# whabacivch/GC-SLAM

Measured on AMD Instinct MI355X. Metric: scans/sec (14-step pipeline) at 64k pts/scan, higher is better.
Workload: dtype f64

## Files before the change

gc-slam_amd/csrc/gcs_atlas.cpp:

```cpp
#include "gcs_atlas.h"

#include <math.h>

#include <algorithm>
#include <cmath>
#include <thread>
#include <vector>

#include "gcs_math.h"

namespace gcs {
namespace atlas {

void fibonacci(int B, double* dirs) {
  const double pi = 3.141592653589793;
  const double golden = pi * (1.0 + sqrt(5.0));
  for (int i = 0; i < B; ++i) {
    double idx = (double)i + 0.5;
    double phi = acos(1.0 - (2.0 * idx) / (double)B);
    double theta = golden * idx;
    double x = sin(phi) * cos(theta), y = sin(phi) * sin(theta), z = cos(phi);
    double n = sqrt(dot3_exact(x, y, z, x, y, z));
    double d = n + kEpsMass;
    dirs[3 * i] = x / d;
// ... 175 lines not shown
      L[k] = th[k].second;
      const double bd = cos(std::max(th[k].first - rc, 0.0)) + 1e-6;
      F[k] = std::nextafter((float)bd, 2.0f);
    }
  });
  width = 1;
  for (auto& L : lists) width = std::max(width, (int)L.size() + 1);
  width = (width + 3) & ~3;
  pools.assign((size_t)ncell * width, -1);
  for (int c = 0; c < ncell; ++c)
    std::copy(lists[c].begin(), lists[c].end(), pools.begin() + (size_t)c * width);
  if (bounds) {
    bounds->assign((size_t)ncell * width, -2.0f);
    for (int c = 0; c < ncell; ++c)
      std::copy(blists[c].begin(), blists[c].end(), bounds->begin() + (size_t)c * width);
  }
}

namespace {
uint64_t hilbert_d(uint32_t n, uint32_t x, uint32_t y) {
  uint64_t d = 0;
  for (uint32_t s = n / 2; s > 0; s /= 2) {
    uint32_t rx = (x & s) > 0, ry = (y & s) > 0;
    d += (uint64_t)s * s * ((3 * rx) ^ ry);
    if (ry == 0) {
      if (rx == 1) { x = s - 1 - x; y = s - 1 - y; }
      std::swap(x, y);
    }
  }
  return d;
// ... 51 lines not shown
```

gc-slam_amd/csrc/gcs_atlas.h:

```cpp
#pragma once
#include <stdint.h>

#include <vector>

namespace gcs {
namespace atlas {

void fibonacci(int B, double* dirs );
void knn(const double* dirs, int B, int K, int* out );
void nearest(const double* dirs, int B, int nq, const double* q, int* out);
void reverse(const int* knn, int B, int K, std::vector<int>& off, std::vector<int>& idx);
int grid_for_bins(int B);
void cell_pools(const double* dirs, int B, int G, std::vector<int>& pools, int& width,
                std::vector<float>* bounds = nullptr);

void hilbert_order(const double* dirs, int B, std::vector<int>& order);

int tile_sources(const std::vector<int>& rknn_off, const std::vector<int>& rknn, int B, int tile,
                 std::vector<int>& src_off, std::vector<int>& src, std::vector<uint16_t>& local);

}
}
```

gc-slam_amd/csrc/gcs_capi.cpp:

```cpp
#include "gcslam_hip.h"

#include <hip/hip_runtime.h>
#include <math.h>
#include <rccl/rccl.h>
#include <string.h>

#include <algorithm>
#include <atomic>
#include <sys/syscall.h>
#include <unistd.h>
#include <chrono>
#include <condition_variable>
#include <mutex>
#include <thread>
#include <string>
#include <vector>

#include "gcs_atlas.h"
#include "gcs_host.h"
#include "gcs_imu_odom_core.h"
#include "gcs_kernels.h"
#include "gcs_layout.h"
#include "gcs_live.h"
#include "gcs_math.h"
// ... 26 lines not shown
  clk::time_point T0, Tp, T1, Ts, T2;
};

struct gcs_ctx {
  gcs_config cfg{};
  int B = 0, cap = 0, K = 0, G = 0, pool_width = 0, ncell = 0, max_raw = 0;
  hipStream_t stream = nullptr;
  bool own_stream = false;
  std::string err;
  double* d_bin_dirs = nullptr;
  int* d_knn = nullptr;
  int* d_rknn_off = nullptr;
  int* d_rknn = nullptr;
  int* d_pools = nullptr;
  float* d_pool_bound = nullptr;
  std::vector<double> dirs_host;
  std::vector<int> knn_host;
  std::vector<int> order, inv;
  int* d_bin_ref = nullptr;
  int* d_tile_src_off = nullptr;
  int* d_tile_src = nullptr;
  uint16_t* d_rknn_local = nullptr;
  int max_tile_src = 0;
  int tile_bins = 64;
  int tile_shift = 6;
  PointRec* d_recs = nullptr;
  double* d_iz = nullptr;
  bool iz_valid = false;
  double *d_live_p0 = nullptr, *d_live_w = nullptr, *d_live_t = nullptr;
  gcs_scan_state* scan_st = nullptr;
// ... 300 lines not shown
    std::vector<uint16_t> local;
    c->max_tile_src = atlas::tile_sources(off, idx, B, c->tile_bins, src_off, src, local);
    if (c->max_tile_src > bins_max_tile_sources(c->tile_bins))
      return fail(c, GCS_ERR_ARG, "bin atlas too irregular for the tiled bin kernel (tile source list too long)");
    for (int b0 = 0; b0 < B; b0 += c->tile_bins)
      if (off[std::min(B, b0 + c->tile_bins)] - off[b0] > bins_max_tile_entries(c->tile_bins))
        return fail(c, GCS_ERR_ARG, "bin atlas too irregular for the tiled bin kernel (tile reverse-kNN list too long)");
    c->G = atlas::grid_for_bins(B);
    c->ncell = 6 * c->G * c->G;
    std::vector<float> pbound;
    atlas::cell_pools(c->dirs_host.data(), B, c->G, pools, c->pool_width, &pbound);
    if (int rc = upload(c, c->d_pool_bound, pbound)) return rc;
    for (int& id : pools)
      if (id >= 0) id = c->inv[id];
    if (int rc = upload(c, c->d_pools, pools)) return rc;
    HIPCHK(c, hipMemcpy(c->d_knn, knn_dev.data(), knn_dev.size() * sizeof(int), hipMemcpyHostToDevice));
    HIPCHK(c, hipMemcpy(c->d_rknn_off, off.data(), off.size() * sizeof(int), hipMemcpyHostToDevice));
    HIPCHK(c, hipMemcpy(c->d_rknn, idx.data(), idx.size() * sizeof(int), hipMemcpyHostToDevice));
    if (int rc = upload(c, c->d_tile_src_off, src_off)) return rc;
    if (int rc = upload(c, c->d_tile_src, src)) return rc;
    if (int rc = upload(c, c->d_rknn_local, local)) return rc;
  }
  HIPCHK(c, hipStreamSynchronize(nullptr));
  return GCS_OK;
}

int submit_budget(gcs_ctx* c, const BudgetArgs& ba, int nblk, hipStream_t s);

int stage_budget(gcs_ctx* c, const double* w, int n_raw, bool toggle = true, bool self = false) {
  if (n_raw < 0 || n_raw > c->max_raw) return fail(c, GCS_ERR_ARG, "n_points exceeds max_raw_points");
// ... 64 lines not shown
  a.cap = c->cap;
  a.t0 = t0;
  a.t1 = t1;
  memcpy(a.xi, xi, 6 * sizeof(double));
  memcpy(a.origin, c->cfg.lidar_origin, 3 * sizeof(double));
  a.tau = c->cfg.tau;
  a.bin_dirs = c->d_bin_dirs;
  a.n_bins = c->B;
  a.knn = c->d_knn;
  a.k = c->K;
  a.pools = c->d_pools;
  a.pool_bound = c->d_pool_bound;
  a.bin_ref = c->d_bin_ref;
  a.pool_width = c->pool_width;
  a.grid = c->G;
  a.recs = c->d_recs;
  a.keys = c->d_keys;
  a.slots = c->d_slots;
  a.counts = c->d_counts;
  if (c->use_direct) {
    a.members = c->d_members;
    a.capb = c->capb_eff;
    a.flags = c->d_flags;
    a.tile_shift = c->tile_shift;
    a.overflow = c->d_err + 2;
  }
  a.budget_partials = c->budget_self ? nullptr : c->d_partials;
  a.budget_blocks = c->budget_self ? 0 : c->budget_blocks;
  a.mass_rows = c->budget_self ? c->d_mass_rows : nullptr;
  c->recs_deferred = c->budget_self && c->cfg.mode == GCS_MODE_SCALE && !deskew_only;
// ... 17 lines not shown
  if (deskew_only) {
    a.n_bins = 0;
    a.nearest_out = nullptr;
    a.members = nullptr;
  }
  c->pts_blocks = points_blocks(c->cap, scale);
  c->pts_fold_pending = scale && fold_later;
  MirrorArgs mir{};
  if (to_host && !c->pts_fold_pending) {
    mir.mirror = c->d_scalars_mirror;
    mir.err = c->d_err;
    mir.seq = ++c->mirror_seq;
    mir.torn = c->mirror_torn;
  }
  HIPCHK(c, launch_points(a, scale, c->d_part_pts, c->pts_blocks, !c->pts_fold_pending, s, ev.e0, ev.e1,
                          c->legacy_points, mir));
  return GCS_OK;
}

BinKernelArgs bin_args(gcs_ctx* c) {
  BinKernelArgs b{};
  b.recs = c->d_recs;
  b.perm = c->d_perm;
  if (c->use_direct) {
    b.members = c->d_members;
    b.capb = c->capb_eff;
  }
  b.starts = c->d_starts;
  b.counts = c->d_counts;
  b.flags = c->d_flags;
  b.tile_dirty = c->d_tile_dirty;
// ... 446 lines not shown
  auto bad = [&](hipError_t e) {
    if (e != hipSuccess) {
      gcs_ctx_destroy(c);
      return true;
    }
    return false;
  };
  if (bad(hipSetDevice(cfg->device))) return GCS_ERR_HIP;
  if (bad(hipStreamCreateWithFlags(&c->stream, hipStreamNonBlocking))) return GCS_ERR_HIP;
  c->own_stream = true;
  if (bad(hipStreamCreateWithFlags(&c->push_stream, hipStreamNonBlocking))) return GCS_ERR_HIP;
  if (bad(hipEventCreateWithFlags(&c->ev_push, hipEventDisableTiming))) return GCS_ERR_HIP;
  if (bad(hipEventCreateWithFlags(&c->ev_stages, hipEventDisableTiming))) return GCS_ERR_HIP;
  if (const char* pt = getenv("GCSLAM_PUSH_THREAD")) c->push_async = atoi(pt) != 0;
  if (const char* sb = getenv("GCSLAM_SORTED_BUCKETS")) c->direct_buckets = atoi(sb) == 0;
  const size_t B = c->B, cap = c->cap;
  if (bad(hipMalloc(&c->d_bin_dirs, B * 4 * sizeof(double)))) return GCS_ERR_HIP;
  if (bad(hipMalloc(&c->d_recs, cap * sizeof(PointRec)))) return GCS_ERR_HIP;
  if (bad(hipMalloc(&c->d_iz, cap * sizeof(double)))) return GCS_ERR_HIP;
  if (bad(hipMalloc(&c->d_live_p0, 3 * cap * sizeof(double)))) return GCS_ERR_HIP;
  if (bad(hipMalloc(&c->d_live_w, cap * sizeof(double)))) return GCS_ERR_HIP;
  if (bad(hipMalloc(&c->d_live_t, cap * sizeof(double)))) return GCS_ERR_HIP;
  if (bad(hipMalloc(&c->d_nearest, cap * sizeof(int)))) return GCS_ERR_HIP;
  if (bad(hipMalloc(&c->d_scan, B * SF_COUNT * sizeof(double)))) return GCS_ERR_HIP;
  if (bad(hipMalloc(&c->d_map, B * MF_COUNT * sizeof(double)))) return GCS_ERR_HIP;
  if (bad(hipMalloc(&c->d_derived, B * MD_COUNT * sizeof(double)))) return GCS_ERR_HIP;
  if (bad(hipMemset(c->d_map, 0, B * MF_COUNT * sizeof(double)))) return GCS_ERR_HIP;
  if (bad(hipMemset(c->d_scan, 0, B * SF_COUNT * sizeof(double)))) return GCS_ERR_HIP;
  if (bad(hipMalloc(&c->d_touched, B))) return GCS_ERR_HIP;
  c->partials_len = std::max<size_t>({partials_need(kRedBlocks, 24), partials_need(pt_blocks(c->B), 13), partials_need(bins_scale_blocks(c->B, c->tile_bins), bins_partial_nv()),
// ... 90 lines not shown
}

int gcs_ctx_destroy(gcs_ctx* c) {
  if (!c) return GCS_OK;
  if (c->push_thread.joinable()) {
    (void)push_wait(c);
    {
      std::lock_guard<std::mutex> lk(c->push_mu);
      c->push_stop.store(true);
    }
    c->push_cv.notify_one();
    c->push_thread.join();
  }
  if (c->push_stream) (void)hipStreamSynchronize(c->push_stream);
  if (c->stream) (void)hipStreamSynchronize(c->stream);
  void* ptrs[] = {c->d_gate_xi, c->d_members, c->d_bin_dirs, c->d_knn, c->d_rknn_off, c->d_rknn, c->d_pools, c->d_pool_bound, c->d_recs, c->d_iz, c->d_live_p0, c->d_live_w, c->d_live_t, c->d_keys, c->d_slots,
                  c->d_sorted, c->d_nearest, c->d_counts, c->d_starts, c->d_perm, c->d_flags_buf[0], c->d_touched,
                  c->d_tile_dirty, c->d_tile_order, c->d_tile_work, c->d_bins_part, c->d_tickets,
                  c->d_bin_ref, c->d_tile_src_off, c->d_tile_src, c->d_rknn_local, c->d_part_pts, c->d_mass_rows, c->d_part_push, c->d_parse_flag,
                  c->d_scan, c->d_map, c->d_derived, c->d_bin_partials, c->d_partials, c->d_scalars};
  for (void* p : ptrs)
    if (p) (void)hipFree(p);
  if (c->h_scalars) (void)hipHostFree(c->h_scalars);
  if (c->d_err) (void)hipFree(c->d_err);
  if (c->h_gate) (void)hipHostFree(c->h_gate);
  if (c->h_preint_in) (void)hipHostFree(c->h_preint_in);
  if (c->h_preint_out) (void)hipHostFree(c->h_preint_out);
  if (c->comm_stream) {
    (void)hipStreamSynchronize(c->comm_stream);
    (void)hipStreamDestroy(c->comm_stream);
  }
// ... 153 lines not shown
  if (int rc = push_wait(c)) return rc;
  if (c->push_stream) HIPCHK(c, hipStreamSynchronize(c->push_stream));
  HIPCHK(c, hipStreamSynchronize(c->stream));
  const size_t B = c->B;
  int rc = 0;
  if ((rc = dev_fnv(c, c->d_scan, B * SF_COUNT * sizeof(double), &out[0]))) return rc;
  if ((rc = dev_fnv(c, c->d_map, B * MF_COUNT * sizeof(double), &out[1]))) return rc;
  if ((rc = dev_fnv(c, c->d_derived, B * MD_COUNT * sizeof(double), &out[2]))) return rc;
  if ((rc = dev_fnv(c, c->d_touched, B, &out[3]))) return rc;
  const size_t nflags = c->d_flags_buf[0] ? 2 * ((B + bins_scale_blocks(c->B, c->tile_bins) + 15) & ~(size_t)15) : 0;
  if ((rc = dev_fnv(c, c->d_flags_buf[0], nflags, &out[4]))) return rc;
  const size_t npart = c->d_bins_part ? (size_t)bins_scale_blocks(c->B, c->tile_bins) * partial_stride(bins_partial_nv()) : 0;
  if ((rc = dev_fnv(c, c->d_bins_part, npart * sizeof(double), &out[5]))) return rc;
  if ((rc = dev_fnv(c, c->d_scalars, SC_COUNT * sizeof(double), &out[6]))) return rc;
  out[7] = fnv1a(c->h_scalars, SC_COUNT * sizeof(double));
  return GCS_OK;
}

int gcs_ctx_enable_timing(gcs_ctx* c, int32_t stage_mask) {
  if (!c) return GCS_ERR_ARG;
  if (stage_mask && c->ev[0].empty())
    for (int st = 0; st < kStages; ++st) {
      c->ev[st].resize(2 * gcs_ctx::kEvRing, nullptr);
      for (hipEvent_t& e : c->ev[st]) HIPCHK(c, hipEventCreateWithFlags(&e, hipEventDisableSystemFence));
    }
  c->timing_mask = (uint32_t)stage_mask;
  return GCS_OK;
}

int gcs_ctx_stage_times(gcs_ctx* c, double* ms_sum, int64_t* counts, int32_t reset) {
// ... 1844 lines not shown
  Belief a;
  to_host_belief(*b, a);
  host::mean_world_pose(a, pose6);
  return GCS_OK;
}
int gcs_fibonacci_atlas(int32_t B, double* dirs) {
  if (B < 1 || !dirs) return GCS_ERR_ARG;
  atlas::fibonacci(B, dirs);
  return GCS_OK;
}
int gcs_knn_table(int32_t B, const double* dirs, int32_t k, int32_t* knn) {
  if (B < 1 || k < 1 || k > B || !dirs || !knn) return GCS_ERR_ARG;
  atlas::knn(dirs, B, k, knn);
  return GCS_OK;
}
int gcs_nearest_bins(int32_t B, const double* dirs, int32_t nq, const double* q, int32_t* out) {
  if (B < 1 || nq < 0 || !dirs || (nq && (!q || !out))) return GCS_ERR_ARG;
  atlas::nearest(dirs, B, nq, q, out);
  return GCS_OK;
}

}
```

gc-slam_amd/csrc/gcs_kernels.h:

```cpp
#pragma once
#include <hip/hip_runtime.h>
#include <stddef.h>
#include <stdint.h>

#include "gcs_layout.h"

namespace gcs {


struct ParseArgs {
  const uint8_t* data;
  int n, point_step;
  int off_x, off_y, off_z, off_ring, ring_datatype, off_t, t_datatype;
  double header_stamp;
  double R[9], tb[3];
  double* points;
  double* t;
  double* w;
  uint8_t* ring;
  uint32_t* ns_flag;
};

struct BudgetArgs {
  const double* w;
// ... 27 lines not shown
  const double* timestamps;
  const double* weights;
  int n_raw, n_sel, stride, cap;
  double t0, t1;
  double xi[6];
  double origin[3];
  double tau;
  const double* bin_dirs;
  int n_bins;
  const int* knn;
  int k;
  const int* pools;
  const float* pool_bound;
  const int* bin_ref;
  int pool_width, grid;
  PointRec* recs;
  uint32_t* keys;
  uint32_t* slots;
  uint32_t* counts;
  uint32_t* members;
  int capb;
  uint8_t* flags;
  int tile_shift;
  uint32_t* overflow;
  const double* budget_partials;
  int budget_blocks;
  double2* mass_rows;
  double* scalars;
  double* p0_out;
  double* w_out;
// ... 88 lines not shown
};
struct ImuOdomDevArgs {
  const double* win;
  int m;
  double t_last_scan, t_scan, dt_sec;
  double planar_z_ref, planar_z_sigma, planar_vz_sigma;
  double* out;
  double* host;
  uint64_t* dseq;
};
hipError_t launch_imu_odom(const ImuOdomDevArgs& a, hipStream_t s);
hipError_t launch_gate(const uint64_t* gate, uint64_t seq, double* xi_out, uint32_t* err, hipStream_t s);
hipError_t launch_payload_out(const double* src, double* host, int n, uint64_t* dseq, hipStream_t s);
hipError_t launch_delay(int us, hipStream_t s);
hipError_t launch_points(const PointKernelArgs& a, bool scale, double* partials, int nblk, bool fold, hipStream_t s,
                         hipEvent_t e0, hipEvent_t e1, bool legacy = false, const MirrorArgs& mir = MirrorArgs{});
int scan_tiles(int n_bins);
hipError_t launch_bucketing(const BucketArgs& b, int n, hipStream_t s, hipEvent_t e0, hipEvent_t e1);
int bins_tile_for(long cap, int n_bins);
int bins_scale_blocks(int n_bins, int tile_bins);
int partial_stride(int nv);
size_t partials_need(long nblocks, int nv);
int bins_max_tile_sources(int tile_bins);
int bins_max_tile_entries(int tile_bins);
int bins_partial_nv();
int push_blocks(int n_bins);
hipError_t launch_bins_scale(const BinKernelArgs& a, double* partials, hipStream_t s, hipEvent_t e0, hipEvent_t e1,
                             hipEvent_t f0, hipEvent_t f1);
hipError_t launch_dense(const BinKernelArgs& a, double* bin_partials, double* partials, hipStream_t s, hipEvent_t e0,
                        hipEvent_t e1);
hipError_t launch_mf(const double* scan, const double* map, int B, double* partials, int nblk, double* scalars,
// ... 15 lines not shown
```

gc-slam_amd/csrc/gcs_kernels.hip:

```cpp
#include <hip/hip_runtime.h>


#include "gcs_kernels.h"

#include <hip/hip_ext.h>
#include <string.h>
#include "gcs_layout.h"
#include "gcs_math.h"

namespace gcs {

constexpr int kBlock = 256;
constexpr int kWaves = kBlock / 64;

template <int NV>
__device__ __forceinline__ void wave_sum(double (&v)[NV]) {
#pragma unroll
  for (int off = 32; off >= 1; off >>= 1) {
#pragma unroll
    for (int k = 0; k < NV; ++k) v[k] += __shfl_xor(v[k], off, 64);
  }
}

template <int NV>
// ... 611 lines not shown
    if (a.p0_out) { a.p0_out[3 * (size_t)i] = p0[0]; a.p0_out[3 * (size_t)i + 1] = p0[1]; a.p0_out[3 * (size_t)i + 2] = p0[2]; }
    if (a.w_out) a.w_out[i] = wout;
    if (a.w_budget_out) a.w_budget_out[i] = wb;
    if (a.nearest_out) a.nearest_out[i] = nearest;
    const double wn = a.mass_rows ? wb : wb / (mass_in + kEpsMass);
    acc[0] = 0.0 + wb;
    acc[1] = 0.0 + wn * wn;
    acc[2] = 0.0 + wout;
    acc[3] = 0.0 + H;
    rmax = fmax(rmax, rm);
  }
  block_sum<4>(acc, lds);
  rmax = block_max(rmax, lds);
  double v[5] = {acc[0], acc[1], acc[2], acc[3], rmax};
  store_partials<5>(v, partials, lb);
}

constexpr int kScanThreads = 256;
constexpr int kScanTile = 16 * kScanThreads;
constexpr int kLaneRank = 16;
constexpr int kRankMax = 8192;
constexpr uint32_t kLbAgg = 1u << 30, kLbPre = 2u << 30, kLbVal = (1u << 30) - 1u;

__global__ __launch_bounds__(kScanThreads) void k_scan(const uint32_t* __restrict__ counts, int n, uint32_t* status,
                                                       uint32_t* ticket, uint32_t* start, uint32_t* err,
                                                       uint32_t spin_limit, int inject_fail) {
  constexpr int kSW = kScanThreads / 64;
  __shared__ uint32_t wsum[kSW];
  __shared__ uint32_t s_tile, s_excl;
  const int t = threadIdx.x, lane = t & 63, wid = t >> 6;
// ... 1607 lines not shown
}

hipError_t launch_gate(const uint64_t* gate, uint64_t seq, double* xi_out, uint32_t* err, hipStream_t s) {
  hipLaunchKernelGGL(k_gate, dim3(1), dim3(64), 0, s, gate, seq, xi_out, err);
  return hipGetLastError();
}

constexpr int kPointsMaxBlocks = 4096;
int points_max_blocks() { return kPointsMaxBlocks; }
int points_blocks(long cap, bool scale) {
  const long need = (cap + kBlock - 1) / kBlock;
  return (int)std::max(1L, std::min((long)(scale ? kPointsMaxBlocks : 1024), need));
}

hipError_t launch_points(const PointKernelArgs& a, bool scale, double* partials, int nblk, bool fold, hipStream_t s,
                         hipEvent_t e0, hipEvent_t e1, bool legacy, const MirrorArgs& mir) {
  hipEvent_t ek = fold ? nullptr : e1;
  if (scale && !legacy && (long)nblk * kBlock >= (long)a.cap) {
    switch (a.k) {
      case 8: hipExtLaunchKernelGGL(k_points_lean<8>, dim3(nblk), dim3(kBlock), 0, s, e0, ek, 0, a, partials); break;
      case 16: hipExtLaunchKernelGGL(k_points_lean<16>, dim3(nblk), dim3(kBlock), 0, s, e0, ek, 0, a, partials); break;
      case 32: hipExtLaunchKernelGGL(k_points_lean<32>, dim3(nblk), dim3(kBlock), 0, s, e0, ek, 0, a, partials); break;
      default: return hipErrorInvalidValue;
    }
  } else if (scale) {
    switch (a.k) {
      case 8: hipExtLaunchKernelGGL((k_points<true, 8>), dim3(nblk), dim3(kBlock), 0, s, e0, ek, 0, a, partials); break;
      case 16: hipExtLaunchKernelGGL((k_points<true, 16>), dim3(nblk), dim3(kBlock), 0, s, e0, ek, 0, a, partials); break;
      case 32: hipExtLaunchKernelGGL((k_points<true, 32>), dim3(nblk), dim3(kBlock), 0, s, e0, ek, 0, a, partials); break;
      default: return hipErrorInvalidValue;
    }
  } else if (a.n_bins == 0) {
    hipExtLaunchKernelGGL((k_points<false, 0>), dim3(nblk), dim3(kBlock), 0, s, e0, ek, 0, a, partials);
// ... 99 lines not shown
```

gc-slam_amd/csrc/gcs_layout.h:

```cpp
#pragma once
#include <hip/hip_runtime.h>
#include <stdint.h>

namespace gcs {

enum ScanField : int {
  SF_N = 0,
  SF_SD = 1,
  SF_S = 4,
  SF_PB = 13,
  SF_SIG = 16,
  SF_KAPPA = 25,
  SF_COUNT = 26
};

enum MapField : int {
  MF_SD = 0,
  MF_S = 3,
  MF_ND = 12,
  MF_NP = 13,
  MF_SP = 14,
  MF_SPP = 17,
  MF_COUNT = 26
};
// ... 8 lines not shown

struct PointRec {
  double x, y, z;
  double dx, dy, dz;
  double m;
  double wz;
};
static_assert(sizeof(PointRec) == 64, "point record");

struct PointRec32 {
  double x, y, z;
  double wz;
};
static_assert(sizeof(PointRec32) == 32, "scale-mode point record");

enum Scalar : int {
  SC_MASS_IN = 0,
  SC_MASS_SEL = 1,
  SC_MASS_SCALE = 2,
  SC_DESKEW_WIN = 3,
  SC_BUDGET_W2 = 4,
  SC_DESKEW_WOUT = 5,
  SC_ENTROPY = 6,
  SC_MAXRESP = 7,
  SC_BIN_NSUM = 8,
  SC_BIN_N2SUM = 9,
  SC_BIN_SUPP = 10,
  SC_BIN_PSD = 11,
  SC_BIN_EPSR = 12,
  SC_MF_H = 16,
// ... 29 lines not shown
```

gc-slam_amd/gcslam/_lib.py:

```python

from __future__ import annotations

import ctypes as C
import os

import numpy as np

LIB_NAME = "libgcslam_hip.so"
LIB_PATH = os.path.join(os.path.dirname(os.path.abspath(__file__)), LIB_NAME)

ABI_VERSION = 4
D_Z = 22
CERT_LEN = 64
PAYLOAD_LEN = 840
SCAN_FIELDS = 26
MAP_FIELDS = 26
DERIVED_FIELDS = 16
MODE_DENSE, MODE_SCALE = 0, 1

c_double_p = C.POINTER(C.c_double)
c_int32_p = C.POINTER(C.c_int32)
c_int64_p = C.POINTER(C.c_int64)


# ... 423 lines not shown
    ("gcs_pmap_recency_inflate", C.c_int, [C.c_void_p, c_int32_p, C.c_int32, C.c_int64, C.c_double, C.c_double,
                                           c_double_p]),
    ("gcs_pmap_merge_reduce", C.c_int, [C.c_void_p, C.c_int32, C.c_double, C.c_int32, C.c_double, C.c_double,
                                        c_int32_p, c_int32_p, c_int32_p]),
    ("gcs_pmap_map_update", C.c_int, [C.c_void_p, c_int32_p, c_int64_p, C.c_int32, c_double_p, C.c_double, C.c_int64,
                                      c_int64_p, C.POINTER(GcsPmapUpdateConfig), C.POINTER(GcsPmapUpdateInputs),
                                      C.POINTER(GcsPmapUpdateStats), c_int32_p]),
    ("gcs_pmap_export", C.c_int, [C.c_void_p, c_int32_p, c_int64_p, C.c_int32, C.c_int32, C.c_int32, C.c_double,
                                  C.c_double, C.c_int32, C.POINTER(GcsPmapExportOut), c_int32_p, c_int32_p]),
    ("gcs_live_scan", C.c_int, [C.c_void_p, C.c_void_p, C.POINTER(GcsScanBeginOutputs), C.POINTER(GcsLiveArgs),
                                C.POINTER(GcsLiveOutputs), C.POINTER(GcsScanOutputs)]),
    ("gcs_live_collect", C.c_int, [C.c_void_p, C.POINTER(GcsLiveOutputs)]),
    ("gcs_live_scan_camera", C.c_int, [C.c_void_p, C.c_void_p, C.POINTER(GcsScanBeginOutputs), C.POINTER(GcsLiveArgs),
                                       C.c_void_p, C.POINTER(GcsLiveOutputs), C.POINTER(GcsScanOutputs)]),
    ("gcs_ma_hex_stencil", C.c_int, [c_double_p, C.c_double, C.c_int32, C.c_int32, c_int64_p, C.c_int32]),
]

SYMBOLS = [s[0] for s in _SIGS]

_lib = None


_AB_OPTIONAL = ("gcs_ctx_host_split", "gcs_ctx_worker_tid", "gcs_imu_odom_evidence_device",
                "gcs_ctx_host_split_history")


def load():
    global _lib
    if _lib is not None:
        return _lib
# ... 63 lines not shown
```

include/gcslam_hip.h:

```cpp
#ifndef GCSLAM_HIP_H
#define GCSLAM_HIP_H

#include <stddef.h>
#include <stdint.h>

#ifdef __cplusplus
extern "C" {
#endif

#define GCS_ABI_VERSION 4
#define GCS_D_Z 22
#define GCS_SCAN_FIELDS 26
#define GCS_MAP_FIELDS 26
#define GCS_DERIVED_FIELDS 16
#define GCS_PAYLOAD_LEN 840

typedef enum {
  GCS_OK = 0,
  GCS_ERR_ARG = -1,
  GCS_ERR_HIP = -2,
  GCS_ERR_NONFINITE = -3,
  GCS_ERR_STATE = -4
} gcs_status;

// ... 110 lines not shown
#define GCS_DEBUG_SCAN_SPIN_LIMIT 1
#define GCS_DEBUG_INJECT_SCAN_FAIL 2
#define GCS_DEBUG_SORTED_BUCKETS 3
#define GCS_DEBUG_BUCKET_CAPACITY 4
#define GCS_DEBUG_LAUNCH_GATE 5
#define GCS_DEBUG_POINT_KERNEL 6
#define GCS_DEBUG_DEVICE_PREINT 7
#define GCS_DEBUG_PT_CLEAR 8
#define GCS_DEBUG_MIRROR_TORN 9
#define GCS_DEBUG_SENDBUF 10
#define GCS_DEBUG_DEVICE_IMU_ODOM 11
#define GCS_DEBUG_COMBINE_DELAY 12
int gcs_ctx_set_debug(gcs_ctx* ctx, int32_t key, int64_t value);
int gcs_ctx_mirror_stats(gcs_ctx* ctx, int64_t* out );
int gcs_debug_state_checksums(gcs_ctx* ctx, uint64_t* out );
int gcs_ctx_stage_times(gcs_ctx* ctx, double* ms_sum , int64_t* counts ,
                        int32_t reset);
int gcs_ctx_host_split(gcs_ctx* ctx, double* ms_sum , int64_t* n , int32_t reset);
int gcs_ctx_host_split_history(gcs_ctx* ctx, float* out , int32_t n_max, int32_t* n_out);
int64_t gcs_ctx_worker_tid(gcs_ctx* ctx);
int gcs_ctx_set_atlas(gcs_ctx* ctx, const double* dirs_host );
int gcs_ctx_get_atlas(gcs_ctx* ctx, double* dirs_host , int32_t* knn_host );
int gcs_ctx_set_belief(gcs_ctx* ctx, const gcs_belief* b);
int gcs_ctx_get_belief(gcs_ctx* ctx, gcs_belief* b);
int gcs_ctx_set_map(gcs_ctx* ctx, const double* map_host );
int gcs_ctx_get_map(gcs_ctx* ctx, double* map_host , double* derived_host );
int gcs_ctx_get_scan_stats(gcs_ctx* ctx, double* scan_host );
int gcs_ctx_device_arrays(gcs_ctx* ctx, double** scan_dev, double** map_dev, double** derived_dev);
int gcs_ctx_get_bin_order(gcs_ctx* ctx, int32_t* order );
int gcs_ctx_set_iw_state(gcs_ctx* ctx, const double* nu7, const double* Psi7x36);
// ... 563 lines not shown
typedef struct {
  gcs_camsplat_ctx* ctx;
  const gcs_camsplat_inputs* in;
  const void* xyz_dev;
  int32_t point_step, xyz_format, n_points;
  const gcs_camsplat_outputs* src;
  int32_t n_feat;
  gcs_camsplat_outputs* out;
} gcs_live_camera;

int gcs_live_scan_camera(gcs_ctx* ctx, const gcs_scan_inputs* in, gcs_scan_begin_outputs* begin,
                         const gcs_live_args* a, const gcs_live_camera* cam, gcs_live_outputs* lo,
                         gcs_scan_outputs* out);
int gcs_ma_hex_stencil(const double* center3, double h_tile, int32_t radius_xy, int32_t radius_z, int64_t* out,
                       int32_t cap);

#ifdef __cplusplus
}
#endif
#endif
```

Before: 8886.

## Pack kNN candidate rows and pool heads for a new point kernel

```diff
diff --git a/gc-slam_amd/csrc/gcs_atlas.cpp b/gc-slam_amd/csrc/gcs_atlas.cpp
--- a/gc-slam_amd/csrc/gcs_atlas.cpp
+++ b/gc-slam_amd/csrc/gcs_atlas.cpp
@@ -1,12 +1,14 @@
 #include "gcs_atlas.h"
 
 #include <math.h>
+#include <string.h>
 
 #include <algorithm>
 #include <cmath>
 #include <thread>
 #include <vector>
 
+#include "gcs_layout.h"
 #include "gcs_math.h"
 
 namespace gcs {
@@ -213,6 +215,35 @@
     bounds->assign((size_t)ncell * width, -2.0f);
     for (int c = 0; c < ncell; ++c)
       std::copy(blists[c].begin(), blists[c].end(), bounds->begin() + (size_t)c * width);
+  }
+}
+
+void pack_rows(const int* knn_tab, const double* dirs, int dstride, int B, int K, std::vector<uint8_t>& rows) {
+  const size_t stride = (size_t)pack_row_stride(K);
+  rows.assign((size_t)B * stride, 0);
+  for (int b = 0; b < B; ++b) {
+    uint8_t* row = rows.data() + (size_t)b * stride;
+    memcpy(row, knn_tab + (size_t)b * K, (size_t)K * sizeof(int));
+    for (int k = 0; k < K; ++k) {
+      const int id = knn_tab[(size_t)b * K + k];
+      if (id >= 0) memcpy(row + 4 * (size_t)K + 24 * (size_t)k, dirs + (size_t)id * dstride, 24);
+    }
+  }
+}
+
+void pool_heads(const int* pools, const float* bounds, int ncell, int width, const double* dirs, int dstride,
+                std::vector<uint8_t>& heads) {
+  heads.assign((size_t)ncell * kPoolHeadBytes, 0);
+  for (int c = 0; c < ncell; ++c) {
+    uint8_t* hd = heads.data() + (size_t)c * kPoolHeadBytes;
+    const int* pool = pools + (size_t)c * width;
+    int ids[kPoolHeadIds];
+    for (int u = 0; u < kPoolHeadIds; ++u) ids[u] = u < width ? pool[u] : -1;
+    const float bnext = width > kPoolHeadIds ? bounds[(size_t)c * width + kPoolHeadIds] : -2.0f;
+    memcpy(hd, ids, sizeof(ids));
+    memcpy(hd + kPoolHeadBound, &bnext, sizeof(float));
+    for (int u = 0; u < kPoolHeadIds; ++u)
+      if (ids[u] >= 0) memcpy(hd + kPoolHeadDirs + 24 * u, dirs + (size_t)ids[u] * dstride, 24);
   }
 }
 
diff --git a/gc-slam_amd/csrc/gcs_atlas.h b/gc-slam_amd/csrc/gcs_atlas.h
--- a/gc-slam_amd/csrc/gcs_atlas.h
+++ b/gc-slam_amd/csrc/gcs_atlas.h
@@ -14,6 +14,10 @@
 void cell_pools(const double* dirs, int B, int G, std::vector<int>& pools, int& width,
                 std::vector<float>* bounds = nullptr);
 
+void pack_rows(const int* knn, const double* dirs, int dstride, int B, int K, std::vector<uint8_t>& rows);
+void pool_heads(const int* pools, const float* bounds, int ncell, int width, const double* dirs, int dstride,
+                std::vector<uint8_t>& heads);
+
 void hilbert_order(const double* dirs, int B, std::vector<int>& order);
 
 int tile_sources(const std::vector<int>& rknn_off, const std::vector<int>& rknn, int B, int tile,
diff --git a/gc-slam_amd/csrc/gcs_capi.cpp b/gc-slam_amd/csrc/gcs_capi.cpp
--- a/gc-slam_amd/csrc/gcs_capi.cpp
+++ b/gc-slam_amd/csrc/gcs_capi.cpp
@@ -64,6 +64,10 @@
   int* d_rknn = nullptr;
   int* d_pools = nullptr;
   float* d_pool_bound = nullptr;
+  uint8_t* d_cand_rows = nullptr;
+  uint8_t* d_pool_heads = nullptr;
+  bool point_pack = true;
+  int n_cu = 0;
   std::vector<double> dirs_host;
   std::vector<int> knn_host;
   std::vector<int> order, inv;
@@ -394,6 +398,29 @@
     for (int& id : pools)
       if (id >= 0) id = c->inv[id];
     if (int rc = upload(c, c->d_pools, pools)) return rc;
+    for (uint8_t** t : {&c->d_cand_rows, &c->d_pool_heads}) {
+      if (*t) (void)hipFree(*t);
+      *t = nullptr;
+    }
+    if (c->point_pack && (long)c->cap * 5 >= (long)B * 2) {
+      std::vector<uint8_t> rows, heads;
+      atlas::pack_rows(knn_dev.data(), d4.data(), 4, B, K, rows);
+      if (hipMalloc(&c->d_cand_rows, rows.size()) != hipSuccess) {
+        (void)hipGetLastError();
+        c->d_cand_rows = nullptr;
+      } else {
+        HIPCHK(c, hipMemcpy(c->d_cand_rows, rows.data(), rows.size(), hipMemcpyHostToDevice));
+      }
+      if (c->d_cand_rows && rows.size() + (size_t)c->ncell * kPoolHeadBytes <= (size_t)B * 1024) {
+        atlas::pool_heads(pools.data(), pbound.data(), c->ncell, c->pool_width, d4.data(), 4, heads);
+        if (hipMalloc(&c->d_pool_heads, heads.size()) != hipSuccess) {
+          (void)hipGetLastError();
+          c->d_pool_heads = nullptr;
+        } else {
+          HIPCHK(c, hipMemcpy(c->d_pool_heads, heads.data(), heads.size(), hipMemcpyHostToDevice));
+        }
+      }
+    }
     HIPCHK(c, hipMemcpy(c->d_knn, knn_dev.data(), knn_dev.size() * sizeof(int), hipMemcpyHostToDevice));
     HIPCHK(c, hipMemcpy(c->d_rknn_off, off.data(), off.size() * sizeof(int), hipMemcpyHostToDevice));
     HIPCHK(c, hipMemcpy(c->d_rknn, idx.data(), idx.size() * sizeof(int), hipMemcpyHostToDevice));
@@ -488,6 +515,8 @@
   a.bin_ref = c->d_bin_ref;
   a.pool_width = c->pool_width;
   a.grid = c->G;
+  a.cand_rows = c->d_cand_rows;
+  a.pool_heads = c->d_pool_heads;
   a.recs = c->d_recs;
   a.keys = c->d_keys;
   a.slots = c->d_slots;
@@ -535,7 +564,7 @@
     mir.torn = c->mirror_torn;
   }
   HIPCHK(c, launch_points(a, scale, c->d_part_pts, c->pts_blocks, !c->pts_fold_pending, s, ev.e0, ev.e1,
-                          c->legacy_points, mir));
+                          c->legacy_points, mir, c->n_cu));
   return GCS_OK;
 }
 
@@ -1012,6 +1041,8 @@
   if (bad(hipEventCreateWithFlags(&c->ev_stages, hipEventDisableTiming))) return GCS_ERR_HIP;
   if (const char* pt = getenv("GCSLAM_PUSH_THREAD")) c->push_async = atoi(pt) != 0;
   if (const char* sb = getenv("GCSLAM_SORTED_BUCKETS")) c->direct_buckets = atoi(sb) == 0;
+  if (const char* pp = getenv("GCSLAM_POINT_PACK")) c->point_pack = atoi(pp) != 0;
+  if (bad(hipDeviceGetAttribute(&c->n_cu, hipDeviceAttributeMultiprocessorCount, cfg->device))) return GCS_ERR_HIP;
   const size_t B = c->B, cap = c->cap;
   if (bad(hipMalloc(&c->d_bin_dirs, B * 4 * sizeof(double)))) return GCS_ERR_HIP;
   if (bad(hipMalloc(&c->d_recs, cap * sizeof(PointRec)))) return GCS_ERR_HIP;
@@ -1132,7 +1163,7 @@
   }
   if (c->push_stream) (void)hipStreamSynchronize(c->push_stream);
   if (c->stream) (void)hipStreamSynchronize(c->stream);
-  void* ptrs[] = {c->d_gate_xi, c->d_members, c->d_bin_dirs, c->d_knn, c->d_rknn_off, c->d_rknn, c->d_pools, c->d_pool_bound, c->d_recs, c->d_iz, c->d_live_p0, c->d_live_w, c->d_live_t, c->d_keys, c->d_slots,
+  void* ptrs[] = {c->d_gate_xi, c->d_members, c->d_bin_dirs, c->d_knn, c->d_rknn_off, c->d_rknn, c->d_pools, c->d_pool_bound, c->d_cand_rows, c->d_pool_heads, c->d_recs, c->d_iz, c->d_live_p0, c->d_live_w, c->d_live_t, c->d_keys, c->d_slots,
                   c->d_sorted, c->d_nearest, c->d_counts, c->d_starts, c->d_perm, c->d_flags_buf[0], c->d_touched,
                   c->d_tile_dirty, c->d_tile_order, c->d_tile_work, c->d_bins_part, c->d_tickets,
                   c->d_bin_ref, c->d_tile_src_off, c->d_tile_src, c->d_rknn_local, c->d_part_pts, c->d_mass_rows, c->d_part_push, c->d_parse_flag,
@@ -1316,6 +1347,26 @@
   if ((rc = dev_fnv(c, c->d_bins_part, npart * sizeof(double), &out[5]))) return rc;
   if ((rc = dev_fnv(c, c->d_scalars, SC_COUNT * sizeof(double), &out[6]))) return rc;
   out[7] = fnv1a(c->h_scalars, SC_COUNT * sizeof(double));
+  return GCS_OK;
+}
+
+int gcs_debug_point_state(gcs_ctx* c, double* recs, int32_t* nearest, uint32_t* counts, uint32_t* members,
+                          int32_t* info) {
+  if (!c || !info) return GCS_ERR_ARG;
+  if (c->cfg.mode != GCS_MODE_SCALE) return fail(c, GCS_ERR_STATE, "gcs_debug_point_state: scale mode only");
+  if (int rc = push_wait(c)) return rc;
+  if (c->push_stream) HIPCHK(c, hipStreamSynchronize(c->push_stream));
+  HIPCHK(c, hipStreamSynchronize(c->stream));
+  const size_t B = c->B, cap = c->cap;
+  info[0] = c->capb_eff;
+  info[1] = c->direct_buckets && !c->sorted_sticky && c->d_members ? 1 : 0;
+  info[2] = c->d_cand_rows ? (c->d_pool_heads ? 2 : 1) : 0;
+  info[3] = c->d_cand_rows && c->pts_blocks <= c->n_cu ? 1 : 0;
+  if (recs) HIPCHK(c, hipMemcpy(recs, c->d_recs, cap * sizeof(PointRec32), hipMemcpyDeviceToHost));
+  if (nearest) HIPCHK(c, hipMemcpy(nearest, c->d_nearest, cap * sizeof(int), hipMemcpyDeviceToHost));
+  if (counts) HIPCHK(c, hipMemcpy(counts, c->d_counts, B * sizeof(uint32_t), hipMemcpyDeviceToHost));
+  if (members)
+    HIPCHK(c, hipMemcpy(members, c->d_members, B * (size_t)c->capb_eff * sizeof(uint32_t), hipMemcpyDeviceToHost));
   return GCS_OK;
 }
 
@@ -3190,6 +3241,40 @@
   atlas::knn(dirs, B, k, knn);
   return GCS_OK;
 }
+int gcs_debug_cell_pools(int32_t B, const double* dirs, int32_t* dims, int32_t* pools, float* bounds, int64_t cap) {
+  if (B < 1 || !dirs || !dims) return GCS_ERR_ARG;
+  std::vector<int> pl;
+  std::vector<float> bd;
+  int width = 0;
+  const int G = atlas::grid_for_bins(B);
+  atlas::cell_pools(dirs, B, G, pl, width, &bd);
+  dims[0] = G;
+  dims[1] = 6 * G * G;
+  dims[2] = width;
+  if (pools || bounds) {
+    if (!pools || !bounds || cap < (int64_t)pl.size()) return GCS_ERR_ARG;
+    memcpy(pools, pl.data(), pl.size() * sizeof(int));
+    memcpy(bounds, bd.data(), bd.size() * sizeof(float));
+  }
+  return GCS_OK;
+}
+int gcs_debug_atlas_pack(int32_t B, const double* dirs, int32_t k, const int32_t* knn, int32_t n_cells,
+                         int32_t pool_width, const int32_t* pools, const float* bounds, uint8_t* rows, uint8_t* heads) {
+  if (B < 1 || !dirs) return GCS_ERR_ARG;
+  if (rows) {
+    if (k < 1 || !knn) return GCS_ERR_ARG;
+    std::vector<uint8_t> r;
+    atlas::pack_rows(knn, dirs, 3, B, k, r);
+    memcpy(rows, r.data(), r.size());
+  }
+  if (heads) {
+    if (n_cells < 1 || pool_width < 1 || !pools || !bounds) return GCS_ERR_ARG;
+    std::vector<uint8_t> h;
+    atlas::pool_heads(pools, bounds, n_cells, pool_width, dirs, 3, h);
+    memcpy(heads, h.data(), h.size());
+  }
+  return GCS_OK;
+}
 int gcs_nearest_bins(int32_t B, const double* dirs, int32_t nq, const double* q, int32_t* out) {
   if (B < 1 || nq < 0 || !dirs || (nq && (!q || !out))) return GCS_ERR_ARG;
   atlas::nearest(dirs, B, nq, q, out);
diff --git a/gc-slam_amd/csrc/gcs_kernels.h b/gc-slam_amd/csrc/gcs_kernels.h
--- a/gc-slam_amd/csrc/gcs_kernels.h
+++ b/gc-slam_amd/csrc/gcs_kernels.h
@@ -65,6 +65,8 @@
   const float* pool_bound;
   const int* bin_ref;
   int pool_width, grid;
+  const uint8_t* cand_rows;
+  const uint8_t* pool_heads;
   PointRec* recs;
   uint32_t* keys;
   uint32_t* slots;
@@ -183,7 +185,8 @@
 hipError_t launch_payload_out(const double* src, double* host, int n, uint64_t* dseq, hipStream_t s);
 hipError_t launch_delay(int us, hipStream_t s);
 hipError_t launch_points(const PointKernelArgs& a, bool scale, double* partials, int nblk, bool fold, hipStream_t s,
-                         hipEvent_t e0, hipEvent_t e1, bool legacy = false, const MirrorArgs& mir = MirrorArgs{});
+                         hipEvent_t e0, hipEvent_t e1, bool legacy = false, const MirrorArgs& mir = MirrorArgs{},
+                         int n_cu = 0);
 int scan_tiles(int n_bins);
 hipError_t launch_bucketing(const BucketArgs& b, int n, hipStream_t s, hipEvent_t e0, hipEvent_t e1);
 int bins_tile_for(long cap, int n_bins);
diff --git a/gc-slam_amd/csrc/gcs_kernels.hip b/gc-slam_amd/csrc/gcs_kernels.hip
--- a/gc-slam_amd/csrc/gcs_kernels.hip
+++ b/gc-slam_amd/csrc/gcs_kernels.hip
@@ -649,6 +649,249 @@
   rmax = block_max(rmax, lds);
   double v[5] = {acc[0], acc[1], acc[2], acc[3], rmax};
   store_partials<5>(v, partials, lb);
+}
+
+template <int KC, bool WIDE>
+__device__ __forceinline__ void points_pack_body(const PointKernelArgs& a, double* partials) {
+  constexpr int CG = (WIDE || KC < 8) ? KC : 8;
+  constexpr int EG = 4;
+  static_assert(KC % CG == 0 && KC % 4 == 0, "candidate groups");
+  __shared__ double lds[kWaves * 5];
+  __shared__ double s_mass[2];
+  const int nb = (int)gridDim.x;
+  const int lb = (nb & 7) ? (int)blockIdx.x : (int)(blockIdx.x & 7u) * (nb >> 3) + (int)(blockIdx.x >> 3);
+  static_assert(kBlock * 4 >= 1024, "k_budget launches at most 1024 blocks: four rows per thread");
+  double2 brow[4];
+#pragma unroll
+  for (int k = 0; k < 4; ++k) {
+    const int r = threadIdx.x + k * kBlock;
+    brow[k] = r < a.budget_blocks ? *(const double2*)(a.budget_partials + (size_t)r * pstride<2>())
+                                  : make_double2(0.0, 0.0);
+  }
+  const int i = lb * kBlock + (int)threadIdx.x;
+  const bool live = i < a.cap;
+  const bool valid = live && i < a.n_sel;
+  double p[3] = {0.0, 0.0, 0.0}, t = 0.0, w_raw = 0.0;
+  if (valid) {
+    const size_t src = (size_t)i * (size_t)a.stride;
+    if (a.xyz_f64) {
+      const double* rec = (const double*)(a.xyz + src * (size_t)a.point_step);
+      p[0] = rec[0]; p[1] = rec[1]; p[2] = rec[2];
+    } else {
+      const float* rec = (const float*)(a.xyz + src * (size_t)a.point_step);
+      p[0] = (double)rec[0]; p[1] = (double)rec[1]; p[2] = (double)rec[2];
+    }
+    t = a.timestamps[src];
+    w_raw = a.weights[src];
+  }
+  double bsum[2] = {0.0, 0.0};
+  if (a.mass_rows) {
+    if (valid) {
+      const size_t src = (size_t)i * (size_t)a.stride;
+      bsum[0] = w_raw;
+      for (int q = 1; q < a.stride && src + q < (size_t)a.n_raw; ++q) bsum[0] += a.weights[src + q];
+      bsum[1] = w_raw;
+    }
+  } else {
+#pragma unroll
+    for (int k = 0; k < 4; ++k) {
+      bsum[0] += brow[k].x;
+      bsum[1] += brow[k].y;
+    }
+  }
+  double p0[3], d[3], win;
+  {
+    double xi[6];
+#pragma unroll
+    for (int k = 0; k < 6; ++k) xi[k] = a.xi_dev ? a.xi_dev[k] : a.xi[k];
+    const double denom = a.t1 - a.t0 > 1e-12 ? a.t1 - a.t0 : 1e-12;
+    const double alpha = (t - a.t0) / denom;
+    deskew_point(alpha, xi, p, p0);
+    win = smooth_window(t, a.t0, a.t1, kTimeWarpSigmaFrac * denom);
+    ray_dir(p0[0], p0[1], p0[2], a.origin, d);
+  }
+  int nearest = 0;
+  if (!(d[0] == 0.0 && d[1] == 0.0 && d[2] == 0.0)) {
+    const size_t cell = (size_t)cube_cell(d[0], d[1], d[2], a.grid);
+    const size_t prow = cell * a.pool_width;
+    const int4* pool = (const int4*)(a.pools + prow);
+    const float* pbound = a.pool_bound + prow;
+    const int nq = a.pool_width >> 2;
+    double best = -INFINITY;
+    int q = 0;
+    bool more = true;
+    if (a.pool_heads) {
+      const uint8_t* hd = a.pool_heads + cell * (size_t)kPoolHeadBytes;
+      const int4 u0 = *(const int4*)hd;
+      const int4 u1 = *(const int4*)(hd + 16);
+      const float bnext = *(const float*)(hd + kPoolHeadBound);
+      double f[3 * kPoolHeadIds];
+#pragma unroll
+      for (int u = 0; u < 3 * kPoolHeadIds; u += 2) {
+        const double2 v = *(const double2*)(hd + kPoolHeadDirs + 8 * u);
+        f[u] = v.x; f[u + 1] = v.y;
+      }
+      const int ids[8] = {u0.x, u0.y, u0.z, u0.w, u1.x, u1.y, u1.z, u1.w};
+      double s[8];
+#pragma unroll
+      for (int u = 0; u < 8; ++u) {
+        const double sv = dot3_exact(d[0], d[1], d[2], f[3 * u], f[3 * u + 1], f[3 * u + 2]);
+        s[u] = ids[u] >= 0 ? sv : -INFINITY;
+      }
+#pragma unroll
+      for (int u = 0; u < 8; ++u) {
+        if (s[u] > best) {
+          best = s[u];
+          nearest = ids[u];
+        } else if (s[u] == best && ids[u] >= 0 && a.bin_ref[ids[u]] < a.bin_ref[nearest]) {
+          nearest = ids[u];
+        }
+      }
+      more = !(u1.w < 0 || (best > 0.0 && (double)bnext < best));
+      q = 2;
+    }
+    for (; more && q < nq; q += 2) {
+      const int4 u0 = pool[q];
+      const int4 u1 = q + 1 < nq ? pool[q + 1] : make_int4(-1, -1, -1, -1);
+      const float bnext = q + 2 < nq ? pbound[4 * (q + 2)] : -2.0f;
+      const int ids[8] = {u0.x, u0.y, u0.z, u0.w, u1.x, u1.y, u1.z, u1.w};
+      double s[8];
+#pragma unroll
+      for (int u = 0; u < 8; ++u) {
+        const double* bp = a.bin_dirs + 4 * (size_t)(ids[u] >= 0 ? ids[u] : 0);
+        const double2 xy = *(const double2*)bp;
+        const double sv = dot3_exact(d[0], d[1], d[2], xy.x, xy.y, bp[2]);
+        s[u] = ids[u] >= 0 ? sv : -INFINITY;
+      }
+#pragma unroll
+      for (int u = 0; u < 8; ++u) {
+        if (s[u] > best) {
+          best = s[u];
+          nearest = ids[u];
+        } else if (s[u] == best && ids[u] >= 0 && a.bin_ref[ids[u]] < a.bin_ref[nearest]) {
+          nearest = ids[u];
+        }
+      }
+      if (u1.w < 0 || (best > 0.0 && (double)bnext < best)) break;
+    }
+  }
+  const uint8_t* row = a.cand_rows + (size_t)nearest * (size_t)pack_row_stride(KC);
+  int cid[KC];
+#pragma unroll
+  for (int k = 0; k < KC; k += 4) {
+    const int4 c4 = *(const int4*)(row + 4 * k);
+    cid[k] = c4.x; cid[k + 1] = c4.y; cid[k + 2] = c4.z; cid[k + 3] = c4.w;
+  }
+  double e[KC];
+  double m = -INFINITY;
+  uint32_t sl = 0u;
+#pragma unroll
+  for (int k0 = 0; k0 < KC; k0 += CG) {
+    const double2* g = (const double2*)(row + 4 * KC + 24 * k0);
+    if (k0 > 0) __asm__ volatile("" : "+v"(g) : "v"(m));
+    double f[3 * CG];
+#pragma unroll
+    for (int u = 0; u < 3 * CG; u += 2) {
+      const double2 v = g[u >> 1];
+      f[u] = v.x; f[u + 1] = v.y;
+    }
+    if (k0 == 0 && valid) sl = atomicAdd(a.counts + nearest, 1u);
+#pragma unroll
+    for (int k = 0; k < CG; ++k) {
+      e[k0 + k] = dot3_exact(d[0], d[1], d[2], f[3 * k], f[3 * k + 1], f[3 * k + 2]);
+      m = fmax(m, e[k0 + k]);
+    }
+    if (CG < KC) __builtin_amdgcn_sched_barrier(0);
+  }
+  const double inv_tau = 1.0 / a.tau;
+  double Z = 0.0, sxe = 0.0;
+#pragma unroll
+  for (int k = 0; k < KC; ++k) {
+    const double x = (e[k] - m) * inv_tau;
+    e[k] = exp(x);
+    Z += e[k];
+    sxe += x * e[k];
+    if (!WIDE && (k & (EG - 1)) == EG - 1) __builtin_amdgcn_sched_barrier(0);
+  }
+  const double iz = 1.0 / Z;
+  double corr = 0.0, rm = 0.0;
+#pragma unroll
+  for (int k = 0; k < KC; ++k) {
+    const double r = e[k] * iz;
+    corr += r * __builtin_amdgcn_rcp(r + kEpsMass);
+    rm = fmax(rm, r);
+  }
+  const double H = log(Z) - sxe * iz - kEpsMass * corr;
+  if (valid) {
+    if (a.members) {
+      if (sl < (uint32_t)a.capb) a.members[(size_t)nearest * a.capb + sl] = (uint32_t)i;
+      else *a.overflow = 1u;
+      if (sl == 0u) {
+        const int ts = a.tile_shift;
+        uint8_t* tf = a.flags + a.n_bins;
+#pragma unroll
+        for (int k = 0; k < KC; ++k) {
+          a.flags[cid[k]] = 1;
+          tf[cid[k] >> ts] = 1;
+        }
+      }
+    } else {
+      a.slots[i] = sl;
+    }
+  }
+  if (live && !a.members) a.keys[i] = valid ? (uint32_t)nearest : (uint32_t)a.n_bins;
+  block_sum<2>(bsum, lds);
+  if (threadIdx.x == 0) {
+    if (a.mass_rows) {
+      a.mass_rows[lb] = make_double2(bsum[0], bsum[1]);
+      s_mass[0] = 0.0;
+      s_mass[1] = 1.0;
+    } else {
+      s_mass[0] = bsum[0];
+      s_mass[1] = bsum[0] / (bsum[1] + kEpsMass);
+      if (lb == 0) {
+        a.scalars[SC_MASS_IN] = bsum[0];
+        a.scalars[SC_MASS_SEL] = bsum[1];
+        a.scalars[SC_MASS_SCALE] = s_mass[1];
+      }
+    }
+  }
+  __syncthreads();
+  const double mass_scale = s_mass[1], mass_in = s_mass[0];
+  double acc[4] = {0.0, 0.0, 0.0, 0.0};
+  double rmax = -INFINITY;
+  if (live) {
+    const double wb = w_raw * mass_scale;
+    const double wout = wb * win;
+    reinterpret_cast<double4*>(a.recs)[i] = make_double4(p0[0], p0[1], p0[2], wout * iz);
+    if (a.t_out) a.t_out[i] = t;
+    if (a.iz_out) a.iz_out[i] = iz;
+    if (a.p0_out) { a.p0_out[3 * (size_t)i] = p0[0]; a.p0_out[3 * (size_t)i + 1] = p0[1]; a.p0_out[3 * (size_t)i + 2] = p0[2]; }
+    if (a.w_out) a.w_out[i] = wout;
+    if (a.w_budget_out) a.w_budget_out[i] = wb;
+    if (a.nearest_out) a.nearest_out[i] = nearest;
+    const double wn = a.mass_rows ? wb : wb / (mass_in + kEpsMass);
+    acc[0] = 0.0 + wb;
+    acc[1] = 0.0 + wn * wn;
+    acc[2] = 0.0 + wout;
+    acc[3] = 0.0 + H;
+    rmax = fmax(rmax, rm);
+  }
+  block_sum<4>(acc, lds);
+  rmax = block_max(rmax, lds);
+  double v[5] = {acc[0], acc[1], acc[2], acc[3], rmax};
+  store_partials<5>(v, partials, lb);
+}
+
+template <int KC>
+__global__ __launch_bounds__(kBlock) __attribute__((amdgpu_waves_per_eu(4)))
+void k_points_pack(PointKernelArgs a, double* partials) {
+  points_pack_body<KC, false>(a, partials);
+}
+
+template <int KC>
+__global__ __launch_bounds__(kBlock) void k_points_pack_wide(PointKernelArgs a, double* partials) {
+  points_pack_body<KC, true>(a, partials);
 }
 
 constexpr int kScanThreads = 256;
@@ -2286,9 +2529,25 @@
 }
 
 hipError_t launch_points(const PointKernelArgs& a, bool scale, double* partials, int nblk, bool fold, hipStream_t s,
-                         hipEvent_t e0, hipEvent_t e1, bool legacy, const MirrorArgs& mir) {
+                         hipEvent_t e0, hipEvent_t e1, bool legacy, const MirrorArgs& mir, int n_cu) {
   hipEvent_t ek = fold ? nullptr : e1;
-  if (scale && !legacy && (long)nblk * kBlock >= (long)a.cap) {
+  if (scale && !legacy && a.cand_rows && (long)nblk * kBlock >= (long)a.cap) {
+    if (nblk <= n_cu) {
+      switch (a.k) {
+        case 8: hipExtLaunchKernelGGL(k_points_pack_wide<8>, dim3(nblk), dim3(kBlock), 0, s, e0, ek, 0, a, partials); break;
+        case 16: hipExtLaunchKernelGGL(k_points_pack_wide<16>, dim3(nblk), dim3(kBlock), 0, s, e0, ek, 0, a, partials); break;
+        case 32: hipExtLaunchKernelGGL(k_points_pack_wide<32>, dim3(nblk), dim3(kBlock), 0, s, e0, ek, 0, a, partials); break;
+        default: return hipErrorInvalidValue;
+      }
+    } else {
+      switch (a.k) {
+        case 8: hipExtLaunchKernelGGL(k_points_pack<8>, dim3(nblk), dim3(kBlock), 0, s, e0, ek, 0, a, partials); break;
+        case 16: hipExtLaunchKernelGGL(k_points_pack<16>, dim3(nblk), dim3(kBlock), 0, s, e0, ek, 0, a, partials); break;
+        case 32: hipExtLaunchKernelGGL(k_points_pack<32>, dim3(nblk), dim3(kBlock), 0, s, e0, ek, 0, a, partials); break;
+        default: return hipErrorInvalidValue;
+      }
+    }
+  } else if (scale && !legacy && (long)nblk * kBlock >= (long)a.cap) {
     switch (a.k) {
       case 8: hipExtLaunchKernelGGL(k_points_lean<8>, dim3(nblk), dim3(kBlock), 0, s, e0, ek, 0, a, partials); break;
       case 16: hipExtLaunchKernelGGL(k_points_lean<16>, dim3(nblk), dim3(kBlock), 0, s, e0, ek, 0, a, partials); break;
diff --git a/gc-slam_amd/csrc/gcs_layout.h b/gc-slam_amd/csrc/gcs_layout.h
--- a/gc-slam_amd/csrc/gcs_layout.h
+++ b/gc-slam_amd/csrc/gcs_layout.h
@@ -46,6 +46,12 @@
 };
 static_assert(sizeof(PointRec32) == 32, "scale-mode point record");
 
+constexpr int kPoolHeadIds = 8;
+constexpr int kPoolHeadBytes = 256;
+constexpr int kPoolHeadBound = 32;
+constexpr int kPoolHeadDirs = 64;
+__host__ __device__ constexpr int pack_row_stride(int K) { return (28 * K + 63) & ~63; }
+
 enum Scalar : int {
   SC_MASS_IN = 0,
   SC_MASS_SEL = 1,
diff --git a/gc-slam_amd/gcslam/_lib.py b/gc-slam_amd/gcslam/_lib.py
--- a/gc-slam_amd/gcslam/_lib.py
+++ b/gc-slam_amd/gcslam/_lib.py
@@ -461,6 +461,10 @@
     ("gcs_live_scan_camera", C.c_int, [C.c_void_p, C.c_void_p, C.POINTER(GcsScanBeginOutputs), C.POINTER(GcsLiveArgs),
                                        C.c_void_p, C.POINTER(GcsLiveOutputs), C.POINTER(GcsScanOutputs)]),
     ("gcs_ma_hex_stencil", C.c_int, [c_double_p, C.c_double, C.c_int32, C.c_int32, c_int64_p, C.c_int32]),
+    ("gcs_debug_point_state", C.c_int, [C.c_void_p, C.c_void_p, C.c_void_p, C.c_void_p, C.c_void_p, c_int32_p]),
+    ("gcs_debug_cell_pools", C.c_int, [C.c_int32, c_double_p, c_int32_p, C.c_void_p, C.c_void_p, C.c_int64]),
+    ("gcs_debug_atlas_pack", C.c_int, [C.c_int32, c_double_p, C.c_int32, c_int32_p, C.c_int32, C.c_int32, c_int32_p,
+                                       C.c_void_p, C.c_void_p, C.c_void_p]),
 ]
 
 SYMBOLS = [s[0] for s in _SIGS]
diff --git a/include/gcslam_hip.h b/include/gcslam_hip.h
--- a/include/gcslam_hip.h
+++ b/include/gcslam_hip.h
@@ -148,6 +148,8 @@
 int gcs_ctx_set_debug(gcs_ctx* ctx, int32_t key, int64_t value);
 int gcs_ctx_mirror_stats(gcs_ctx* ctx, int64_t* out );
 int gcs_debug_state_checksums(gcs_ctx* ctx, uint64_t* out );
+int gcs_debug_point_state(gcs_ctx* ctx, double* recs, int32_t* nearest, uint32_t* counts, uint32_t* members,
+                          int32_t* info );
 int gcs_ctx_stage_times(gcs_ctx* ctx, double* ms_sum , int64_t* counts ,
                         int32_t reset);
 int gcs_ctx_host_split(gcs_ctx* ctx, double* ms_sum , int64_t* n , int32_t reset);
@@ -741,6 +743,11 @@
                          gcs_scan_outputs* out);
 int gcs_ma_hex_stencil(const double* center3, double h_tile, int32_t radius_xy, int32_t radius_z, int64_t* out,
                        int32_t cap);
+int gcs_debug_cell_pools(int32_t n_bins, const double* dirs, int32_t* dims , int32_t* pools, float* bounds,
+                         int64_t cap);
+int gcs_debug_atlas_pack(int32_t n_bins, const double* dirs, int32_t k, const int32_t* knn, int32_t n_cells,
+                         int32_t pool_width, const int32_t* pools, const float* bounds, uint8_t* rows,
+                         uint8_t* heads);
 
 #ifdef __cplusplus
 }
```

Result: slower. 8702 (-2.1%).
